# pr0g/ToyMeshPathTracer

Hardware: NVIDIA B200
Metric: Mrays/s (primary+bounce+shadow) (higher is better)
Workload: dtype f32

## Files before the change

toymeshpathtracer_b200/csrc/integrator.cuh:

```cuda
#pragma once
#include "bvh.cuh"

namespace integ {

constexpr int kMaxDepth = 10;
constexpr float kMinT = 0.001f;
constexpr float kMaxT = 1.0e7f;

struct Camera {
    ex::V3 origin, lowerLeftCorner, horizontal, vertical, u, v, w;
    float lensRadius;
};

TMPT_HD void camera_get_ray(const Camera& c, float s, float t, uint32_t& rng, ex::V3& o, ex::V3& d) {
    float px, py;
    ex::random_in_unit_disk(rng, px, py);
    const float rdx = ex::mul(c.lensRadius, px), rdy = ex::mul(c.lensRadius, py);
    const ex::V3 offset = ex::add(ex::muls(c.u, rdx), ex::muls(c.v, rdy));
    o = ex::add(c.origin, offset);
    d = ex::normalize(ex::sub(ex::sub(ex::add(ex::add(c.lowerLeftCorner, ex::muls(c.horizontal, s)), ex::muls(c.vertical, t)), c.origin), offset));
}

TMPT_HD void primary_ray(const Camera& c, int x, int y, float invW, float invH, uint32_t& rng, ex::V3& o, ex::V3& d) {
    const float fv = ex::mul(ex::add((float)y, ex::random_float01(rng)), invH);
    const float fu = ex::mul(ex::add((float)x, ex::random_float01(rng)), invW);
    camera_get_ray(c, fu, fv, rng, o, d);
}

TMPT_HD ex::V3 sky(ex::V3 dir) {
    const float t = ex::mul(0.5f, ex::add(dir.y, 1.0f));
    const float a = ex::sub(1.0f, t);
    return ex::muls(ex::add(ex::v3(ex::mul(1.0f, a), ex::mul(1.0f, a), ex::mul(1.0f, a)), ex::muls(ex::v3(0.5f, 0.7f, 1.0f), t)), 0.5f);
}

TMPT_HD float sun_term(ex::V3 normal, ex::V3 rayDir, ex::V3 lightDir) {
    const ex::V3 nl = ex::dot(normal, rayDir) < 0.0f ? normal : ex::neg(normal);
    return fmaxf(0.0f, ex::dot(lightDir, nl));
}

TMPT_HD ex::V3 scatter_dir(ex::V3 pos, ex::V3 normal, uint32_t& rng) {
    const ex::V3 target = ex::add(ex::add(pos, normal), ex::random_unit_vector(rng));
    return ex::normalize(ex::sub(target, pos));
}

TMPT_HD ex::V3 unwind_step(float k, ex::V3 color) {
    const ex::V3 albedo = ex::v3(0.7f, 0.7f, 0.7f);
    const ex::V3 kLightColor = ex::v3(0.7f, 0.6f, 0.5f);
    const ex::V3 light = ex::add(ex::v3(0.0f, 0.0f, 0.0f), ex::muls(ex::mulv(albedo, kLightColor), k));
    return ex::add(light, ex::mulv(albedo, color));
}

TMPT_HD uchar4 resolve_pixel(ex::V3 sum, float sppRecip) {
    const ex::V3 c = ex::muls(sum, sppRecip);
    uchar4 px;
    px.x = ex::quantise(ex::sqrt_rn(c.x));
    px.y = ex::quantise(ex::sqrt_rn(c.y));
    px.z = ex::quantise(ex::sqrt_rn(c.z));
    px.w = 255;
    return px;
}

struct FirstHit {
    int id;
    float t;
    ex::V3 normal;
};

template <bool STATS = false, bool FAR = true, bool AOV = false, class Stack, class Scene>
TMPT_HD ex::V3 trace_path(Stack& stack, const Scene& sc, const Camera& cam, ex::V3 o, ex::V3 d, ex::V3 lightDir, uint32_t& rng,
                          unsigned long long& rays, bvh::TravStats* stats = nullptr, FirstHit* first = nullptr) {
    float kk[kMaxDepth];
    int depth = 0;
    ex::V3 color = ex::v3(0.0f, 0.0f, 0.0f);
    if (AOV) first->id = -1;
    while (depth < kMaxDepth) {
        ++rays;
        const bvh::HitRec h = bvh::traverse_with<false, STATS, FAR>(stack, sc, o, d, kMinT, kMaxT, stats);
        if (h.id < 0) { color = sky(d); break; }
        ex::V3 pos, normal;
        bvh::hit_payload(sc, h.id, h.u, h.v, pos, normal);
        if (AOV && depth == 0) { first->id = h.id; first->t = h.t; first->normal = normal; }
        ++rays;
#if defined(TMPT_SUN_ONLY) && TMPT_SUN_ONLY
        const bool shadowed = bvh::sun_occluded<STATS>(sc, pos, lightDir, kMinT, kMaxT, stats);
#else
        const bool shadowed = sc.sun.n > 0 ? bvh::sun_occluded<STATS>(sc, pos, lightDir, kMinT, kMaxT, stats)
                                           : bvh::traverse_with<true, STATS, FAR>(stack, sc, pos, lightDir, kMinT, kMaxT, stats).id >= 0;
#endif
        kk[depth] = shadowed ? 0.0f : sun_term(normal, d, lightDir);
        d = scatter_dir(pos, normal, rng);
        o = pos;
        ++depth;
    }
    for (int i = depth - 1; i >= 0; --i) color = unwind_step(kk[i], color);
    return color;
}

constexpr int kMaxChunkSamples = 8;
TMPT_HD int chunk_len(int spp) {
    const int c = spp / 32;
    return c < 1 ? 1 : c > kMaxChunkSamples ? kMaxChunkSamples : c;
}
TMPT_HD int chunk_count(int spp) { const int c = chunk_len(spp); return (spp + c - 1) / c; }

struct AovSums {
    ex::V3 normal;
    float t, hits;
    int id0;
};
TMPT_HD void aov_clear(AovSums& a) { a.normal = ex::v3(0.0f, 0.0f, 0.0f); a.t = 0.0f; a.hits = 0.0f; a.id0 = -1; }
TMPT_HD void aov_add_hit(AovSums& a, ex::V3 normal, float t) { a.normal = ex::add(a.normal, normal); a.t = ex::add(a.t, t); a.hits = ex::add(a.hits, 1.0f); }

TMPT_HD float4 radiance_of(ex::V3 sum, float sppRecip) {
    const ex::V3 c = ex::muls(sum, sppRecip);
    return make_float4(c.x, c.y, c.z, 1.0f);
}
TMPT_HD float4 normal_of(ex::V3 normalSum, float hits, float sppRecip) {
    const ex::V3 n = ex::muls(normalSum, sppRecip);
    return make_float4(n.x, n.y, n.z, ex::mul(hits, sppRecip));
}
TMPT_HD float depth_of(float tSum, float hits) { return hits > 0.0f ? ex::divf(tSum, hits) : ex::u2f(0x7F800000u); }

template <bool STATS = false, bool FAR = true, bool AOV = false, class Stack, class Scene>
TMPT_HD ex::V3 render_chunk(Stack& stack, const Scene& sc, const Camera& cam, int x, int y, int chunk, int width, int height, int spp, int len, ex::V3 lightDir,
                            unsigned long long& rays, bvh::TravStats* stats = nullptr, AovSums* aov = nullptr) {
    const float invW = ex::divf(1.0f, (float)width), invH = ex::divf(1.0f, (float)height);
    uint32_t rng = ex::chunk_seed((uint32_t)chunk, (uint32_t)y * (uint32_t)width + (uint32_t)x, (uint32_t)width * (uint32_t)height);
    ex::V3 sum = ex::v3(0.0f, 0.0f, 0.0f);
    const int s0 = chunk * len, s1 = s0 + len < spp ? s0 + len : spp;
    if (AOV) aov_clear(*aov);
    for (int s = s0; s < s1; ++s) {
        ex::V3 o, d;
        primary_ray(cam, x, y, invW, invH, rng, o, d);
        FirstHit fh;
        sum = ex::add(sum, trace_path<STATS, FAR, AOV>(stack, sc, cam, o, d, lightDir, rng, rays, stats, &fh));
        if (AOV) {
            if (s == s0) aov->id0 = fh.id;
            if (fh.id >= 0) aov_add_hit(*aov, fh.normal, fh.t);
        }
    }
    return sum;
}

TMPT_HD void adaptive_add_chunk(ex::V3 chunkSum, uint32_t& n, float& mean, float& m2) {
    const float y = ex::mul(ex::add(ex::add(ex::mul(0.2126f, chunkSum.x), ex::mul(0.7152f, chunkSum.y)), ex::mul(0.0722f, chunkSum.z)), 0.125f);
    n += 1u;
    const float delta = ex::sub(y, mean);
    mean = ex::add(mean, ex::divf(delta, (float)n));
    m2 = ex::add(m2, ex::mul(delta, ex::sub(y, mean)));
}
TMPT_HD bool adaptive_converged(uint32_t n, float mean, float m2, float tolerance, int minChunks) {
    if (tolerance == 0.0f || n < (uint32_t)minChunks) return false;
    const float a = ex::mul(m2, 65025.0f);
    const float b = ex::mul(ex::mul(ex::mul((float)n, (float)(n - 1u)), ex::mul(4.0f, fmaxf(mean, 0x1p-16f))), ex::mul(tolerance, tolerance));
    return !(a > b);
}

template <bool STATS = false, bool AOV = false, class Scene>
TMPT_HD uchar4 render_pixel(const Scene& sc, const Camera& cam, int x, int y, int width, int height, int spp, ex::V3 lightDir,
                            unsigned long long& rays, ex::V3* outLinear = nullptr, bvh::TravStats* stats = nullptr, AovSums* aov = nullptr) {
    const float sppRecip = ex::divf(1.0f, (float)spp);
    ex::V3 sum = ex::v3(0.0f, 0.0f, 0.0f);
    bvh::LocalStack stack;
    if (AOV) aov_clear(*aov);
    for (int c = 0; c < chunk_count(spp); ++c) {
        AovSums ca;
        sum = ex::add(sum, render_chunk<STATS, true, AOV>(stack, sc, cam, x, y, c, width, height, spp, chunk_len(spp), lightDir, rays, stats, &ca));
        if (AOV) {
            if (c == 0) aov->id0 = ca.id0;
            aov->normal = ex::add(aov->normal, ca.normal); aov->t = ex::add(aov->t, ca.t); aov->hits = ex::add(aov->hits, ca.hits);
        }
    }
    if (outLinear) *outLinear = ex::muls(sum, sppRecip);
    return resolve_pixel(sum, sppRecip);
}

}
```

toymeshpathtracer_b200/csrc/kernels.cu:

```cuda
#include <cooperative_groups.h>
#include <cuda_runtime.h>

#include <atomic>
#include <chrono>
#include <cmath>
#include <cstdarg>
#include <cstdio>
#include <cstdlib>
#include <cstring>
#include <mutex>
#include <new>
#include <string>
#include <vector>

#include "build_logic.cuh"
#include "common.h"
#include "denoise.cuh"
#include "integrator.cuh"
#ifndef TMPT_EXPERIMENTS
#define TMPT_EXPERIMENTS 0
#endif

namespace tmpt {
static thread_local std::string g_err;
// ... 538 lines not shown
                if (h.id >= 0) {
                    if (outT) outT[ray] = h.t;
                    if (outPos || outNormal) {
                        ex::V3 pos, nrm;
                        bvh::hit_payload(sc, h.id, h.u, h.v, pos, nrm);
                        if (outPos) { outPos[ray * 3] = pos.x; outPos[ray * 3 + 1] = pos.y; outPos[ray * 3 + 2] = pos.z; }
                        if (outNormal) { outNormal[ray * 3] = nrm.x; outNormal[ray * 3 + 1] = nrm.y; outNormal[ray * 3 + 2] = nrm.z; }
                    }
                }
            }
            ray = -1;
        }
    }
}
#endif

struct RenderParams {
    bvh::SceneView sc;
    integ::Camera cam;
    ex::V3 lightDir;
    int width, height, spp;
    int stripeRows, rank, world, ownedRows;
    int localWidth;
    int tilesX, numTiles;
    int chunks;
    int chunk0, chunkLen;
    int useAccum;
    float4* sumBuf;
    int bandRow0, bandRows;
    float4* accum;
    uchar4* outStripes;
    uchar4* frame;
    float4* radiance;
    float4* normal;
    float* depth;
    int32_t* triangle;
    unsigned long long* rayCount;
    uint32_t* tileCounter;
    unsigned long long* laneCounter;
    unsigned long long* stats;
    const uint2* list;
    int listLen;
};

__device__ __forceinline__ int owned_row_to_global(int r, int stripeRows, int rank, int world) {
    const int ls = r / stripeRows;
    return (ls * world + rank) * stripeRows + (r - ls * stripeRows);
}
__device__ __forceinline__ bool local_to_global(int xl, int r, int stripeRows, int rank, int world, int width, int& x, int& y) {
    if (stripeRows > 0) {
        x = xl;
        y = owned_row_to_global(r, stripeRows, rank, world);
        return true;
    }
    y = r;
    int t0 = (rank - (r >> 2)) % world;
    t0 += t0 < 0 ? world : 0;
    x = ((t0 + (xl >> 3) * world) << 3) + (xl & 7);
    return x < width;
}

template <int SSTACK, int THREADS>
struct RenderStack {
    using type = bvh::SmemStack<SSTACK, THREADS>;
    static __device__ __forceinline__ type make() {
        extern __shared__ unsigned long long smemStack[];
        return type::make(smemStack, threadIdx.x);
    }
};
template <int THREADS>
struct RenderStack<0, THREADS> {
    using type = bvh::LocalStack;
    static __device__ __forceinline__ type make() { return type(); }
};

#ifndef TMPT_SSTACK
#define TMPT_SSTACK 0
#endif
#ifndef TMPT_TUNE_CFG
#define TMPT_TUNE_CFG 0
#endif
constexpr int kSStack = TMPT_SSTACK;

template <bool STATS, int THREADS, int MINB, int SSTACK, bool FAR = false, bool AOV = false, bool LIST = false>
__global__ void __launch_bounds__(THREADS, MINB) k_render(const RenderParams p) {
    const int lane = threadIdx.x & 31;
    unsigned long long rays = 0;
    bvh::TravStats ts;
    typename RenderStack<SSTACK, THREADS>::type stack = RenderStack<SSTACK, THREADS>::make();
    for (;;) {
        uint32_t tile = 0;
        if (lane == 0) tile = atomicAdd(p.tileCounter, 1u);
        tile = __shfl_sync(0xffffffffu, tile, 0);
        if (tile >= (uint32_t)p.numTiles * (uint32_t)p.chunks) break;
        const int chunk = (int)(tile / (uint32_t)p.numTiles);
        tile -= (uint32_t)chunk * (uint32_t)p.numTiles;
        if (LIST) {
            const uint32_t e = tile * 32u + (uint32_t)lane;
            if (e < (uint32_t)p.listLen) {
                const uint2 en = p.list[e];
                const ex::V3 sum = integ::render_chunk<STATS, FAR>(stack, p.sc, p.cam, (int)(en.x & 0xFFFFu), (int)(en.x >> 16), (int)en.y + chunk, p.width,
                                                                   p.height, 0x7FFFFFFF, integ::kMaxChunkSamples, p.lightDir, rays, &ts);
                __stcs(&p.accum[(size_t)chunk * p.listLen + e], make_float4(sum.x, sum.y, sum.z, 0.0f));
            }
            continue;
        }
        const int tx = (int)(tile % (uint32_t)p.tilesX), ty = (int)(tile / (uint32_t)p.tilesX);
        const int xl = tx * 8 + (lane & 7), rb = ty * 4 + (lane >> 3), r = p.bandRow0 + rb;
        int x, y;
        if (xl < p.localWidth && r < p.ownedRows && local_to_global(xl, r, p.stripeRows, p.rank, p.world, p.width, x, y)) {
            integ::AovSums aov;
            const ex::V3 sum = integ::render_chunk<STATS, FAR, AOV>(stack, p.sc, p.cam, x, y, p.chunk0 + chunk, p.width, p.height, p.spp, p.chunkLen, p.lightDir, rays, &ts, &aov);
            if (AOV && p.triangle && p.chunk0 + chunk == 0) p.triangle[(size_t)y * p.width + x] = aov.id0;
            if (p.useAccum) {
                const size_t a = ((size_t)chunk * p.bandRows + rb) * p.localWidth + xl;
                __stcs(&p.accum[a], make_float4(sum.x, sum.y, sum.z, AOV ? aov.hits : 0.0f));
                if (AOV) __stcs(&p.accum[a + (size_t)p.chunks * p.bandRows * p.localWidth], make_float4(aov.normal.x, aov.normal.y, aov.normal.z, aov.t));
            } else {
                const uchar4 px = integ::resolve_pixel(sum, ex::divf(1.0f, (float)p.spp));
                if (p.frame) p.frame[(size_t)y * p.width + x] = px;
                else p.outStripes[(size_t)r * p.localWidth + xl] = px;
            }
        }
    }
    if (STATS) flush_stats(p.stats, rays, ts, 0);
    for (int o = 16; o > 0; o >>= 1) rays += __shfl_xor_sync(0xffffffffu, rays, o);
    if (lane == 0 && rays) atomicAdd(p.rayCount, rays);
}

#if TMPT_EXPERIMENTS
enum : int { ST_WALK = 0, ST_HIT = 1, ST_SHADOW_DONE = 2, ST_PATH_END = 3, ST_NEED_ITEM = 4, ST_IDLE = 5 };

template <bool STATS, int THREADS, int MINB, int TA, int TB>
__global__ void __launch_bounds__(THREADS, MINB) k_render_regen(const RenderParams p) {
    constexpr unsigned FULL = 0xffffffffu;
    const int lane = threadIdx.x & 31;
    bvh::LocalStack stack;
    float kk[integ::kMaxDepth];
    bvh::WalkState w;
    bvh::TravStats ts;
    w.any = false; w.best.id = -1;
    unsigned long long rays = 0;
    int state = ST_NEED_ITEM;
    bool exhausted = false;
    uint32_t rng = 0;
    int depth = 0, s = 0, sEnd = 0, x = 0, y = 0, xl = 0, rb = 0, chunk = 0;
    ex::V3 sum = ex::v3(0.0f, 0.0f, 0.0f), nd = ex::v3(0.0f, 0.0f, 0.0f);
    float sunk = 0.0f;
    const float invW = ex::divf(1.0f, (float)p.width), invH = ex::divf(1.0f, (float)p.height);
    const unsigned long long totalItems = (unsigned long long)p.numTiles * (unsigned long long)p.chunks * 32ull;
    for (;;) {
        const unsigned notWalking = __ballot_sync(FULL, state != ST_WALK);
        if (notWalking) {
            bool newRay = false, newAny = false;
            ex::V3 no = ex::v3(0.0f, 0.0f, 0.0f), ndir = no;
            const unsigned adv = __ballot_sync(FULL, state == ST_HIT || state == ST_SHADOW_DONE);
            if (adv && (__popc(adv) >= TA || notWalking == FULL)) {
                if (state == ST_HIT) {
                    ex::V3 pos, normal;
                    bvh::hit_payload(p.sc, w.best.id, w.best.u, w.best.v, pos, normal);
                    sunk = integ::sun_term(normal, w.d, p.lightDir);
                    nd = integ::scatter_dir(pos, normal, rng);
                    no = pos; ndir = p.lightDir; newRay = true; newAny = true;
                } else if (state == ST_SHADOW_DONE) {
                    kk[depth] = w.best.id < 0 ? sunk : 0.0f;
                    ++depth;
                    if (depth < integ::kMaxDepth) { no = w.o; ndir = nd; newRay = true; newAny = false; }
                    else state = ST_PATH_END;
                }
            }
            const unsigned endp = __ballot_sync(FULL, state == ST_PATH_END || state == ST_NEED_ITEM);
            const unsigned busy = __ballot_sync(FULL, state == ST_WALK || newRay);
            if (endp && (__popc(endp) >= TB || busy == 0)) {
                if (state == ST_PATH_END) {
                    ex::V3 color = w.any ? ex::v3(0.0f, 0.0f, 0.0f) : integ::sky(w.d);
                    for (int i = depth - 1; i >= 0; --i) color = integ::unwind_step(kk[i], color);
                    sum = ex::add(sum, color);
                    if (++s == sEnd) {
                        if (p.useAccum) {
                            __stcs(&p.accum[((size_t)chunk * p.bandRows + rb) * p.localWidth + xl], make_float4(sum.x, sum.y, sum.z, 0.0f));
                        } else {
                            const uchar4 px = integ::resolve_pixel(sum, ex::divf(1.0f, (float)p.spp));
                            if (p.frame) p.frame[(size_t)y * p.width + x] = px;
                            else p.outStripes[(size_t)(p.bandRow0 + rb) * p.localWidth + xl] = px;
                        }
                        state = ST_NEED_ITEM;
                    }
                }
                const unsigned want = __ballot_sync(FULL, state == ST_NEED_ITEM);
                if (want) {
                    if (exhausted) {
                        if (state == ST_NEED_ITEM) state = ST_IDLE;
                    } else {
                        const int cnt = __popc(want);
                        unsigned long long base = 0;
                        if (lane == 0) base = atomicAdd(p.laneCounter, (unsigned long long)cnt);
                        base = __shfl_sync(FULL, base, 0);
                        exhausted = base + (unsigned long long)cnt >= totalItems;
                        if (state == ST_NEED_ITEM) {
                            const unsigned long long item = base + (unsigned long long)__popc(want & ((1u << lane) - 1u));
                            if (item >= totalItems) {
                                state = ST_IDLE;
                            } else {
                                const uint32_t wi = (uint32_t)(item >> 5), li = (uint32_t)item & 31u;
                                chunk = (int)(wi / (uint32_t)p.numTiles);
                                const uint32_t tile = wi - (uint32_t)chunk * (uint32_t)p.numTiles;
                                const int tx = (int)(tile % (uint32_t)p.tilesX), ty = (int)(tile / (uint32_t)p.tilesX);
                                xl = tx * 8 + (int)(li & 7u); rb = ty * 4 + (int)(li >> 3);
                                const int r = p.bandRow0 + rb;
                                if (xl < p.localWidth && r < p.ownedRows && local_to_global(xl, r, p.stripeRows, p.rank, p.world, p.width, x, y)) {
// ... 1054 lines not shown
        LAUNCH(k_probe_paths, 32, 128, 0, st, s->view, cam, width, height, s->d_probe);
        CU_TRY(cudaMemcpyAsync(s->h_probe, s->d_probe, 4 * sizeof(unsigned int), cudaMemcpyDeviceToHost, st));
        CU_TRY(cudaEventRecord(s->probeDone, st));
        s->probeCam = *camera; s->probeW = width; s->probeH = height;
        s->probePending = true;
        if (s->probeUsePaths < 0) { CU_TRY(cudaEventSynchronize(s->probeDone)); consume(); }
    }
    *usePaths = s->probeUsePaths == 1;
    return TMPT_OK;
}

extern "C" int tmpt_render_kernel_choice(const tmpt_scene* s, int* kernel, float* escapeFraction) {
    if (!s) return tmpt::fail(TMPT_ERR_ARG, "tmpt_render_kernel_choice: NULL scene");
    if (kernel) *kernel = s->lastUsedPaths;
    if (escapeFraction) *escapeFraction = s->probeEscape;
    return TMPT_OK;
}

static int launch_render(const tmpt_scene* cs, const tmpt_camera* camera, int width, int height, int spp, int stripeRows, int rank, int world,
                         uint8_t* outStripes, uint8_t* frame, unsigned long long* rayCountDev, cudaStream_t st,
                         unsigned long long* statsDev = nullptr, const ProgressivePass* prog = nullptr, const FrameOutputs* outs = nullptr) {
    tmpt_scene* s = const_cast<tmpt_scene*>(cs);
    RenderParams p;
    p.sc = s->view;
    static_assert(sizeof(integ::Camera) == sizeof(tmpt_camera), "camera layout");
    memcpy(&p.cam, camera, sizeof p.cam);
    p.lightDir = host_light_dir();
    p.width = width; p.height = height;
    p.spp = prog ? integ::kMaxChunkSamples * (prog->chunk0 + prog->nChunks) : spp;
    p.stripeRows = stripeRows; p.rank = rank; p.world = world;
    p.ownedRows = tmpt_stripe_rows(height, stripeRows, rank, world);
    p.localWidth = tmpt_local_width(width, stripeRows, world);
    p.tilesX = div_up(p.localWidth, 8);
    p.chunks = prog ? prog->nChunks : host_chunk_count(spp);
    p.chunk0 = prog ? prog->chunk0 : 0;
    p.chunkLen = prog ? integ::kMaxChunkSamples : host_chunk_len(spp);
    p.useAccum = (p.chunks > 1 || prog || (outs && outs->accum())) ? 1 : 0;
    const bool aov = outs && outs->aov();
    p.radiance = outs ? outs->radiance : nullptr;
    p.normal = outs ? outs->normal : nullptr;
    p.depth = outs ? outs->depth : nullptr;
    p.triangle = outs ? outs->triangle : nullptr;
    p.sumBuf = prog ? prog->sum : nullptr;
    p.outStripes = (uchar4*)outStripes;
    p.frame = (uchar4*)frame;
    p.rayCount = rayCountDev;
    p.tileCounter = s->d_tileCounter;
    p.laneCounter = s->d_fetchCounter;
    p.stats = statsDev;
    p.accum = nullptr;
    p.list = nullptr;
    p.listLen = 0;
    const AdaptivePass* ad = prog ? prog->adaptive : nullptr;
    const int units = ad ? ad->listLen : p.ownedRows;
    if (units == 0) return TMPT_OK;
    int bandRows = 0;
    const int prc = ad ? prepare_render_chunks(s, 1, p.chunks, true, units, st, &bandRows, 1, 32)
                       : prepare_render_chunks(s, p.localWidth, p.chunks, p.useAccum != 0, p.ownedRows, st, &bandRows, aov ? 2 : 1);
    if (prc != TMPT_OK) return prc;
    p.accum = s->d_accum;
    static const int cfgEnv = getenv("TMPT_RENDER_CFG") ? atoi(getenv("TMPT_RENDER_CFG")) : 0;
    static const int rk = getenv("TMPT_RENDER_KERNEL") ? atoi(getenv("TMPT_RENDER_KERNEL")) : 0;
#if !TMPT_EXPERIMENTS
    if (rk > 0) return tmpt::fail(TMPT_ERR_ARG, "TMPT_RENDER_KERNEL is set, but this library was built without -DTMPT_EXPERIMENTS=1");
#endif
    if (aov && (statsDev || rk > 0 || (TMPT_TUNE_CFG && cfgEnv >= 4)))
        return tmpt::fail(TMPT_ERR_ARG, "render: AOV outputs need the shipped render kernels (no instrumented pass, TMPT_RENDER_KERNEL or tuning configuration)");
    if (ad && (rk > 0 || (TMPT_TUNE_CFG && cfgEnv >= 4)))
        return tmpt::fail(TMPT_ERR_ARG, "render: adaptive passes need the shipped render kernels (no TMPT_RENDER_KERNEL or tuning configuration)");
    constexpr size_t smemPerThread = (size_t)kSStack * sizeof(unsigned long long);
    if (smemPerThread * 256 > 48 * 1024) {
        CU_TRY(cudaFuncSetAttribute(k_render<false, 256, 4, kSStack>, cudaFuncAttributeMaxDynamicSharedMemorySize, (int)(smemPerThread * 256)));
        CU_TRY(cudaFuncSetAttribute(k_render<true, 256, 4, kSStack>, cudaFuncAttributeMaxDynamicSharedMemorySize, (int)(smemPerThread * 256)));
        CU_TRY(cudaFuncSetAttribute(k_render<false, 256, 4, kSStack, false, true>, cudaFuncAttributeMaxDynamicSharedMemorySize, (int)(smemPerThread * 256)));
        CU_TRY(cudaFuncSetAttribute(k_render<false, 256, 4, kSStack, false, false, true>, cudaFuncAttributeMaxDynamicSharedMemorySize, (int)(smemPerThread * 256)));
    }
    if (smemPerThread * 512 > 48 * 1024) {
        CU_TRY(cudaFuncSetAttribute(k_render<false, 512, 2, kSStack>, cudaFuncAttributeMaxDynamicSharedMemorySize, (int)(smemPerThread * 512)));
        CU_TRY(cudaFuncSetAttribute(k_render<false, 512, 2, kSStack, false, true>, cudaFuncAttributeMaxDynamicSharedMemorySize, (int)(smemPerThread * 512)));
        CU_TRY(cudaFuncSetAttribute(k_render<false, 512, 2, kSStack, false, false, true>, cudaFuncAttributeMaxDynamicSharedMemorySize, (int)(smemPerThread * 512)));
    }
    if (smemPerThread * 1024 > 48 * 1024) {
        CU_TRY(cudaFuncSetAttribute(k_render<false, 1024, 1, kSStack>, cudaFuncAttributeMaxDynamicSharedMemorySize, (int)(smemPerThread * 1024)));
        CU_TRY(cudaFuncSetAttribute(k_render<false, 1024, 1, kSStack, false, true>, cudaFuncAttributeMaxDynamicSharedMemorySize, (int)(smemPerThread * 1024)));
        CU_TRY(cudaFuncSetAttribute(k_render<false, 1024, 1, kSStack, false, false, true>, cudaFuncAttributeMaxDynamicSharedMemorySize, (int)(smemPerThread * 1024)));
    }
    const bool farCamera = s->view.farLimit > 0.0f &&
        std::max(std::max(std::fabs(camera->origin[0]), std::fabs(camera->origin[1])), std::fabs(camera->origin[2])) + std::fabs(camera->lensRadius) >
            0.5f * s->view.farLimit;
    if (farCamera && smemPerThread * 256 > 48 * 1024) {
        CU_TRY(cudaFuncSetAttribute(k_render<false, 256, 4, kSStack, true>, cudaFuncAttributeMaxDynamicSharedMemorySize, (int)(smemPerThread * 256)));
        CU_TRY(cudaFuncSetAttribute(k_render<false, 256, 4, kSStack, true, true>, cudaFuncAttributeMaxDynamicSharedMemorySize, (int)(smemPerThread * 256)));
        CU_TRY(cudaFuncSetAttribute(k_render<false, 256, 4, kSStack, true, false, true>, cudaFuncAttributeMaxDynamicSharedMemorySize, (int)(smemPerThread * 256)));
    }
    bool usePaths = false;
    if (!statsDev && !farCamera && rk == 0 && cfgEnv == 0) {
        const int rc = choose_render_kernel(s, camera, p.cam, width, height, st, &usePaths);
        if (rc != TMPT_OK) return rc;
    }
    if (!statsDev) s->lastUsedPaths = usePaths ? 1 : 0;
    int perSMp256 = 0, perSMp1024 = 0;
    if (usePaths) {
        CU_TRY(cudaOccupancyMaxActiveBlocksPerMultiprocessor(&perSMp256, k_render_paths<256, 4, 8>, 256, 0));
        CU_TRY(cudaOccupancyMaxActiveBlocksPerMultiprocessor(&perSMp1024, k_render_paths<1024, 1, 8>, 1024, 0));
    }
#if TMPT_TUNE_CFG
    if (cfgEnv >= 4 && cfgEnv <= 8) {
        for (p.bandRow0 = 0; p.bandRow0 < p.ownedRows; p.bandRow0 += bandRows) {
            const int rowsHere = std::min(bandRows, p.ownedRows - p.bandRow0);
            p.bandRows = rowsHere;
            p.numTiles = p.tilesX * div_up(rowsHere, 4);
            CU_TRY(cudaMemsetAsync(s->d_tileCounter, 0, sizeof(uint32_t), st));
            if (cfgEnv == 4) LAUNCH((k_render<false, 768, 1, 0>), s->smCount, 768, 0, st, p);
            else if (cfgEnv == 5) LAUNCH((k_render<false, 576, 2, 0>), 2 * s->smCount, 576, 0, st, p);
            else if (cfgEnv == 6) LAUNCH((k_render<false, 640, 2, 0>), 2 * s->smCount, 640, 0, st, p);
            else if (cfgEnv == 7) LAUNCH((k_render<false, 896, 1, 0>), s->smCount, 896, 0, st, p);
            else LAUNCH((k_render<false, 384, 3, 0>), 3 * s->smCount, 384, 0, st, p);
            if (p.useAccum) LAUNCH(k_resolve<false>, div_up((long long)rowsHere * p.localWidth, 256), 256, 0, st, p, rowsHere);
        }
        CU_TRY(cudaGetLastError());
        return TMPT_OK;
    }
#endif
    int perSM256 = 0, perSM512 = 0, perSM1024 = 0;
    CU_TRY(cudaOccupancyMaxActiveBlocksPerMultiprocessor(&perSM256, k_render<false, 256, 4, kSStack>, 256, smemPerThread * 256));
    CU_TRY(cudaOccupancyMaxActiveBlocksPerMultiprocessor(&perSM512, k_render<false, 512, 2, kSStack>, 512, smemPerThread * 512));
    CU_TRY(cudaOccupancyMaxActiveBlocksPerMultiprocessor(&perSM1024, k_render<false, 1024, 1, kSStack>, 1024, smemPerThread * 1024));
    for (int b0 = 0; b0 < units; b0 += bandRows) {
        const int rowsHere = std::min(bandRows, units - b0);
        if (ad) {
            p.list = s->d_adList + b0;
            p.listLen = rowsHere;
            p.numTiles = div_up(rowsHere, 32);
        } else {
            p.bandRow0 = b0;
            p.bandRows = rowsHere;
            p.numTiles = p.tilesX * div_up(rowsHere, 4);
        }
        const long long items = (long long)p.numTiles * p.chunks;
        if (items >= 0xFFFFFFFFll) return tmpt::fail(TMPT_ERR_ARG, "render: too many work items in one band");
        CU_TRY(cudaMemsetAsync(s->d_tileCounter, 0, sizeof(uint32_t), st));
        const int cfg = (statsDev || rk > 0 || farCamera) ? 1 : cfgEnv > 0 ? cfgEnv : (items >= (long long)s->smCount * 32 * 8 && perSM1024 > 0) ? 3 : 1;
        const int threads = cfg == 3 ? 1024 : cfg == 2 ? 512 : 256;
        const int perSM = cfg == 3 ? perSM1024 : cfg == 2 ? perSM512 : perSM256;
        const int grid = (int)std::min<long long>((long long)s->smCount * std::max(perSM, 1), (items + threads / 32 - 1) / (threads / 32));
#if TMPT_EXPERIMENTS
        if (rk > 0 && !statsDev) {
            CU_TRY(cudaMemsetAsync(s->d_fetchCounter, 0, sizeof(unsigned long long), st));
            int perSMr = 0;
#define REGEN_CASE(V, TA, TB)                                                                                        \
            if (rk == V) {                                                                                           \
                CU_TRY(cudaOccupancyMaxActiveBlocksPerMultiprocessor(&perSMr, k_render_regen<false, 256, 4, TA, TB>, 256, 0)); \
                const int gridR = (int)std::min<long long>((long long)s->smCount * std::max(perSMr, 1), (items * 32 + 255) / 256); \
                LAUNCH((k_render_regen<false, 256, 4, TA, TB>), gridR, 256, 0, st, p);                                 \
            } else
            REGEN_CASE(1, 8, 4) REGEN_CASE(2, 4, 2) REGEN_CASE(3, 12, 6) REGEN_CASE(4, 16, 4)
#undef REGEN_CASE
#define PATHS_CASE(V, T, MB, GT)                                                                                       \
            if (rk == V) {                                                                                           \
                CU_TRY(cudaOccupancyMaxActiveBlocksPerMultiprocessor(&perSMr, k_render_paths<T, MB, GT>, T, 0));     \
                const int gridR = (int)std::min<long long>((long long)s->smCount * std::max(perSMr, 1), (items * 32 + T - 1) / T); \
                LAUNCH((k_render_paths<T, MB, GT>), gridR, T, 0, st, p);                                              \
            } else
            PATHS_CASE(5, 256, 4, 1) PATHS_CASE(6, 256, 4, 8) PATHS_CASE(7, 256, 4, 16) PATHS_CASE(8, 1024, 1, 8) PATHS_CASE(9, 1024, 1, 16)
#undef PATHS_CASE
            return tmpt::fail(TMPT_ERR_ARG, "TMPT_RENDER_KERNEL=%d: no such render kernel", rk);
        } else
#endif
        if (usePaths) {
            CU_TRY(cudaMemsetAsync(s->d_fetchCounter, 0, sizeof(unsigned long long), st));
            const bool big = items >= (long long)s->smCount * 32 * 8 && perSMp1024 > 0;
            const int t = big ? 1024 : 256;
            const int gridP = (int)std::min<long long>((long long)s->smCount * std::max(big ? perSMp1024 : perSMp256, 1), (items * 32 + t - 1) / t);
            if (ad) {
                if (big) LAUNCH((k_render_paths<1024, 1, 8, false, true>), gridP, 1024, 0, st, p);
                else LAUNCH((k_render_paths<256, 4, 8, false, true>), gridP, 256, 0, st, p);
            } else if (aov) {
                if (big) LAUNCH((k_render_paths<1024, 1, 8, true>), gridP, 1024, 0, st, p);
                else LAUNCH((k_render_paths<256, 4, 8, true>), gridP, 256, 0, st, p);
            } else if (big) LAUNCH((k_render_paths<1024, 1, 8>), gridP, 1024, 0, st, p);
            else LAUNCH((k_render_paths<256, 4, 8>), gridP, 256, 0, st, p);
        } else if (ad) {
            if (farCamera) LAUNCH((k_render<false, 256, 4, kSStack, true, false, true>), grid, 256, smemPerThread * 256, st, p);
            else if (cfg == 3) LAUNCH((k_render<false, 1024, 1, kSStack, false, false, true>), grid, 1024, smemPerThread * 1024, st, p);
            else if (cfg == 2) LAUNCH((k_render<false, 512, 2, kSStack, false, false, true>), grid, 512, smemPerThread * 512, st, p);
            else LAUNCH((k_render<false, 256, 4, kSStack, false, false, true>), grid, 256, smemPerThread * 256, st, p);
        } else if (aov) {
            if (farCamera) LAUNCH((k_render<false, 256, 4, kSStack, true, true>), grid, 256, smemPerThread * 256, st, p);
            else if (cfg == 3) LAUNCH((k_render<false, 1024, 1, kSStack, false, true>), grid, 1024, smemPerThread * 1024, st, p);
            else if (cfg == 2) LAUNCH((k_render<false, 512, 2, kSStack, false, true>), grid, 512, smemPerThread * 512, st, p);
            else LAUNCH((k_render<false, 256, 4, kSStack, false, true>), grid, 256, smemPerThread * 256, st, p);
        } else if (farCamera && !statsDev) LAUNCH((k_render<false, 256, 4, kSStack, true>), grid, 256, smemPerThread * 256, st, p);
        else if (statsDev) LAUNCH((k_render<true, 256, 4, kSStack>), grid, 256, smemPerThread * 256, st, p);
        else if (cfg == 3) LAUNCH((k_render<false, 1024, 1, kSStack>), grid, 1024, smemPerThread * 1024, st, p);
        else if (cfg == 2) LAUNCH((k_render<false, 512, 2, kSStack>), grid, 512, smemPerThread * 512, st, p);
        else LAUNCH((k_render<false, 256, 4, kSStack>), grid, 256, smemPerThread * 256, st, p);
        if (ad) LAUNCH(k_resolve_adaptive, div_up(rowsHere, 256), 256, 0, st, p, prog->sum, s->d_adN, s->d_adStat, ad->tolerance, ad->minChunks, s->d_adActive);
        else if (p.useAccum && aov) LAUNCH(k_resolve<true>, div_up((long long)rowsHere * p.localWidth, 256), 256, 0, st, p, rowsHere);
        else if (p.useAccum) LAUNCH(k_resolve<false>, div_up((long long)rowsHere * p.localWidth, 256), 256, 0, st, p, rowsHere);
    }
    CU_TRY(cudaGetLastError());
    return TMPT_OK;
}

static int check_render_args(const tmpt_scene* s, const tmpt_camera* camera, int width, int height, int spp) {
    if (!s || !camera) return tmpt::fail(TMPT_ERR_ARG, "render: NULL scene / camera");
    if (width < 1 || width > 10000 || height < 1 || height > 10000 || spp < 1 || spp > 1024)
        return tmpt::fail(TMPT_ERR_ARG, "render: width %d height %d spp %d out of range", width, height, spp);
    return TMPT_OK;
}

extern "C" int tmpt_render_stripes(const tmpt_scene* s, const tmpt_camera* camera, int width, int height, int spp, int stripeRows, int rank,
                                   int worldSize, uint8_t* outStripes, uint8_t* peerFrame, uint64_t* rayCountDev, void* stream) {
    int rc = check_render_args(s, camera, width, height, spp);
    if (rc != TMPT_OK) return rc;
    if (stripeRows < 0 || worldSize < 1 || rank < 0 || rank >= worldSize || (!outStripes && !peerFrame) || !rayCountDev)
        return tmpt::fail(TMPT_ERR_ARG, "tmpt_render_stripes: bad stripe arguments");
    DeviceGuard guard(s->device);
    if (!guard.ok) return tmpt::fail(TMPT_ERR_CUDA, "tmpt_render_stripes: cudaSetDevice(%d) failed", s->device);
    return launch_render(s, camera, width, height, spp, stripeRows, rank, worldSize, outStripes, peerFrame,
                         (unsigned long long*)rayCountDev, stream ? (cudaStream_t)stream : s->stream);
}

static int check_outputs(const char* fn, const tmpt_outputs* out, int mem) {
    if (!out) return tmpt::fail(TMPT_ERR_ARG, "%s: out is NULL", fn);
    if (!out->rgba && !out->radiance && !out->normal && !out->depth && !out->triangle) return tmpt::fail(TMPT_ERR_ARG, "%s: no output requested", fn);
    if (mem != TMPT_HOST && mem != TMPT_DEVICE) return tmpt::fail(TMPT_ERR_ARG, "%s: mem %d", fn, mem);
    return TMPT_OK;
}

static int grow_scratch(void** p, size_t* cap, size_t need) {
    if (*cap >= need) return TMPT_OK;
    cudaFree(*p); *p = nullptr; *cap = 0;
    CU_TRY(cudaMalloc(p, need));
    *cap = need;
    return TMPT_OK;
}

static int render_frame(tmpt_scene* s, const tmpt_camera* camera, int width, int height, int spp, int mem, const tmpt_outputs* out,
                        const ProgressivePass* prog, cudaStream_t st, uint64_t* rayCount, double* seconds) {
    const size_t pixels = (size_t)width * height;
    const size_t bytes[5] = {pixels * 4, pixels * sizeof(float4), pixels * sizeof(float4), pixels * sizeof(float), pixels * sizeof(int32_t)};
    void* user[5] = {out->rgba, out->radiance, out->normal, out->depth, out->triangle};
    void* dev[5] = {out->rgba, out->radiance, out->normal, out->depth, out->triangle};
    if (mem == TMPT_HOST || !out->rgba) {
        int rc = grow_scratch((void**)&s->d_frame, &s->frameBytes, bytes[0]);
        if (rc != TMPT_OK) return rc;
        dev[0] = s->d_frame;
    }
    if (mem == TMPT_HOST)
        for (int k = 1; k < 5; ++k)
            if (user[k]) {
                const int rc = grow_scratch(&s->d_outs[k - 1], &s->outsBytes[k - 1], bytes[k]);
                if (rc != TMPT_OK) return rc;
                dev[k] = s->d_outs[k - 1];
            }
    FrameOutputs f;
    f.radiance = (float4*)dev[1]; f.normal = (float4*)dev[2]; f.depth = (float*)dev[3]; f.triangle = (int32_t*)dev[4];
    AdaptivePass* ad = prog ? prog->adaptive : nullptr;
    int32_t* userSamples = ad ? ad->samples : nullptr;
    if (userSamples && mem == TMPT_HOST) {
        const int rc = grow_scratch((void**)&s->d_samples, &s->samplesBytes, pixels * sizeof(int32_t));
        if (rc != TMPT_OK) return rc;
        ad->samples = s->d_samples;
    }
    const int chunks = prog ? prog->nChunks : host_chunk_count(spp);
    int rc = ad ? prepare_render_chunks(s, 1, chunks, true, (int)pixels, st, nullptr, 1, 32)
                : prepare_render_chunks(s, width, chunks, prog || f.accum(), height, st, nullptr, f.aov() ? 2 : 1);
    if (rc != TMPT_OK) return rc;
    CU_TRY(cudaEventRecord(s->ev0, st));
    CU_TRY(cudaMemsetAsync(s->d_rayCount, 0, sizeof(unsigned long long), st));
    if (ad) {
// ... 414 lines not shown
```

Before: 7780.

## Spill per-path state to shared-memory columns to cut register pressure in render kernel

Moves per-path state (work item, pixel coords, sample counter, depth, RNG, running sum, AOV sums) from registers into a per-thread column of static shared memory, accessed through volatile ld/st.shared, and recomputes pixel indices from the stored item after tracing. Ray counts are packed into a control word and accumulated per warp in shared memory rather than held as 64-bit per-thread counters. The aim is fewer live registers across the BVH traversal so more warps stay resident. In exchange it adds many shared-memory loads and stores per bounce, uses shared memory that may compete with the traversal stack, and disables the 1024-thread AOV configuration.

Result: no change. 7786 (median of 6 runs) (+0.1%).

```diff
diff --git a/toymeshpathtracer_b200/csrc/integrator.cuh b/toymeshpathtracer_b200/csrc/integrator.cuh
--- a/toymeshpathtracer_b200/csrc/integrator.cuh
+++ b/toymeshpathtracer_b200/csrc/integrator.cuh
@@ -60,39 +60,92 @@
     return px;
 }
 
-struct FirstHit {
-    int id;
-    float t;
-    ex::V3 normal;
-};
-
-template <bool STATS = false, bool FAR = true, bool AOV = false, class Stack, class Scene>
-TMPT_HD ex::V3 trace_path(Stack& stack, const Scene& sc, const Camera& cam, ex::V3 o, ex::V3 d, ex::V3 lightDir, uint32_t& rng,
-                          unsigned long long& rays, bvh::TravStats* stats = nullptr, FirstHit* first = nullptr) {
+enum : int {
+    kPsItem = 0,
+    kPsXY,
+    kPsCtl,
+    kPsRng,
+    kPsSum,
+    kPathWords = kPsSum + 3,
+    kPsAovNormal = kPathWords,
+    kPsAovT = kPsAovNormal + 3,
+    kPsAovHits,
+    kPsAovId0,
+    kPathWordsAov
+};
+constexpr uint32_t kCtlRays = 0xFFFFu, kCtlDepthShift = 16, kCtlLeftShift = 20, kCtlFirst = 1u << 28;
+
+template <int WORDS>
+struct RegPathState {
+    uint32_t w[WORDS];
+    TMPT_HD void put(int i, uint32_t v) { w[i] = v; }
+    TMPT_HD uint32_t get(int i) const { return w[i]; }
+};
+template <int STRIDE>
+struct ColumnPathState {
+#ifdef __CUDA_ARCH__
+    uint32_t col;
+    __device__ __forceinline__ void put(int i, uint32_t v) {
+        asm volatile("st.shared.u32 [%0], %1;" ::"r"(col + (uint32_t)(i * STRIDE * 4)), "r"(v) : "memory");
+    }
+    __device__ __forceinline__ uint32_t get(int i) const {
+        uint32_t v;
+        asm volatile("ld.shared.u32 %0, [%1];" : "=r"(v) : "r"(col + (uint32_t)(i * STRIDE * 4)) : "memory");
+        return v;
+    }
+#else
+    uint32_t* col;
+    void put(int i, uint32_t v) { col[(size_t)i * STRIDE] = v; }
+    uint32_t get(int i) const { return col[(size_t)i * STRIDE]; }
+#endif
+};
+template <class PS>
+TMPT_HD void ps_put3(PS& ps, int i, ex::V3 v) { ps.put(i, ex::f2u(v.x)); ps.put(i + 1, ex::f2u(v.y)); ps.put(i + 2, ex::f2u(v.z)); }
+template <class PS>
+TMPT_HD ex::V3 ps_get3(const PS& ps, int i) { return ex::v3(ex::u2f(ps.get(i)), ex::u2f(ps.get(i + 1)), ex::u2f(ps.get(i + 2))); }
+
+template <bool STATS = false, bool FAR = true, bool AOV = false, class PS, class Stack, class Scene>
+TMPT_HD ex::V3 trace_path(PS& ps, Stack& stack, const Scene& sc, ex::V3 o, ex::V3 d, ex::V3 lightDir, bvh::TravStats* stats = nullptr) {
     float kk[kMaxDepth];
-    int depth = 0;
     ex::V3 color = ex::v3(0.0f, 0.0f, 0.0f);
-    if (AOV) first->id = -1;
-    while (depth < kMaxDepth) {
-        ++rays;
+    for (;;) {
         const bvh::HitRec h = bvh::traverse_with<false, STATS, FAR>(stack, sc, o, d, kMinT, kMaxT, stats);
-        if (h.id < 0) { color = sky(d); break; }
+        uint32_t ctl = ps.get(kPsCtl) + 1u;
+        const int depth = (int)((ctl >> kCtlDepthShift) & 15u);
+        if (h.id < 0) {
+            ps.put(kPsCtl, ctl);
+            color = sky(d);
+            break;
+        }
         ex::V3 pos, normal;
         bvh::hit_payload(sc, h.id, h.u, h.v, pos, normal);
-        if (AOV && depth == 0) { first->id = h.id; first->t = h.t; first->normal = normal; }
-        ++rays;
+        if (AOV && depth == 0) {
+            if (ctl & kCtlFirst) ps.put(kPsAovId0, (uint32_t)h.id);
+            ps_put3(ps, kPsAovNormal, ex::add(ps_get3(ps, kPsAovNormal), normal));
+            ps.put(kPsAovT, ex::f2u(ex::add(ex::u2f(ps.get(kPsAovT)), h.t)));
+            ps.put(kPsAovHits, ex::f2u(ex::add(ex::u2f(ps.get(kPsAovHits)), 1.0f)));
+        }
+        ps.put(kPsCtl, ctl + 1u);
+        const float k = sun_term(normal, d, lightDir);
 #if defined(TMPT_SUN_ONLY) && TMPT_SUN_ONLY
         const bool shadowed = bvh::sun_occluded<STATS>(sc, pos, lightDir, kMinT, kMaxT, stats);
 #else
         const bool shadowed = sc.sun.n > 0 ? bvh::sun_occluded<STATS>(sc, pos, lightDir, kMinT, kMaxT, stats)
                                            : bvh::traverse_with<true, STATS, FAR>(stack, sc, pos, lightDir, kMinT, kMaxT, stats).id >= 0;
 #endif
-        kk[depth] = shadowed ? 0.0f : sun_term(normal, d, lightDir);
+        ctl = ps.get(kPsCtl);
+        const int dk = (int)((ctl >> kCtlDepthShift) & 15u);
+        kk[dk] = shadowed ? 0.0f : k;
+        uint32_t rng = ps.get(kPsRng);
         d = scatter_dir(pos, normal, rng);
+        ps.put(kPsRng, rng);
         o = pos;
-        ++depth;
-    }
-    for (int i = depth - 1; i >= 0; --i) color = unwind_step(kk[i], color);
+        ps.put(kPsCtl, ctl + (1u << kCtlDepthShift));
+        if (dk + 1 == kMaxDepth) break;
+    }
+    const uint32_t ctl = ps.get(kPsCtl);
+    for (int i = (int)((ctl >> kCtlDepthShift) & 15u) - 1; i >= 0; --i) color = unwind_step(kk[i], color);
+    ps.put(kPsCtl, ctl & ~(15u << kCtlDepthShift));
     return color;
 }
 
@@ -121,25 +174,43 @@
 }
 TMPT_HD float depth_of(float tSum, float hits) { return hits > 0.0f ? ex::divf(tSum, hits) : ex::u2f(0x7F800000u); }
 
+template <bool STATS = false, bool FAR = true, bool AOV = false, class PS, class Stack, class Scene>
+TMPT_HD ex::V3 render_chunk(PS& ps, Stack& stack, const Scene& sc, const Camera& cam, int x, int y, int chunk, int width, int height, int spp, int len,
+                            ex::V3 lightDir, unsigned long long& rays, bvh::TravStats* stats = nullptr, AovSums* aov = nullptr) {
+    ps.put(kPsXY, (uint32_t)x | ((uint32_t)y << 16));
+    ps.put(kPsRng, ex::chunk_seed((uint32_t)chunk, (uint32_t)y * (uint32_t)width + (uint32_t)x, (uint32_t)width * (uint32_t)height));
+    const int s0 = chunk * len, s1 = s0 + len < spp ? s0 + len : spp;
+    ps.put(kPsCtl, s1 > s0 ? ((uint32_t)(s1 - s0) << kCtlLeftShift) | kCtlFirst : 0u);
+    ps_put3(ps, kPsSum, ex::v3(0.0f, 0.0f, 0.0f));
+    if (AOV) {
+        AovSums a;
+        aov_clear(a);
+        ps_put3(ps, kPsAovNormal, a.normal);
+        ps.put(kPsAovT, ex::f2u(a.t)); ps.put(kPsAovHits, ex::f2u(a.hits)); ps.put(kPsAovId0, (uint32_t)a.id0);
+    }
+    while (ps.get(kPsCtl) >> kCtlLeftShift) {
+        const float invW = ex::divf(1.0f, (float)width), invH = ex::divf(1.0f, (float)height);
+        const uint32_t xy = ps.get(kPsXY);
+        uint32_t rng = ps.get(kPsRng);
+        ex::V3 o, d;
+        primary_ray(cam, (int)(xy & 0xFFFFu), (int)(xy >> 16), invW, invH, rng, o, d);
+        ps.put(kPsRng, rng);
+        const ex::V3 c = trace_path<STATS, FAR, AOV>(ps, stack, sc, o, d, lightDir, stats);
+        ps_put3(ps, kPsSum, ex::add(ps_get3(ps, kPsSum), c));
+        ps.put(kPsCtl, (ps.get(kPsCtl) - (1u << kCtlLeftShift)) & ~kCtlFirst);
+    }
+    rays += ps.get(kPsCtl) & kCtlRays;
+    if (AOV) {
+        aov->normal = ps_get3(ps, kPsAovNormal);
+        aov->t = ex::u2f(ps.get(kPsAovT)); aov->hits = ex::u2f(ps.get(kPsAovHits)); aov->id0 = (int)ps.get(kPsAovId0);
+    }
+    return ps_get3(ps, kPsSum);
+}
 template <bool STATS = false, bool FAR = true, bool AOV = false, class Stack, class Scene>
 TMPT_HD ex::V3 render_chunk(Stack& stack, const Scene& sc, const Camera& cam, int x, int y, int chunk, int width, int height, int spp, int len, ex::V3 lightDir,
                             unsigned long long& rays, bvh::TravStats* stats = nullptr, AovSums* aov = nullptr) {
-    const float invW = ex::divf(1.0f, (float)width), invH = ex::divf(1.0f, (float)height);
-    uint32_t rng = ex::chunk_seed((uint32_t)chunk, (uint32_t)y * (uint32_t)width + (uint32_t)x, (uint32_t)width * (uint32_t)height);
-    ex::V3 sum = ex::v3(0.0f, 0.0f, 0.0f);
-    const int s0 = chunk * len, s1 = s0 + len < spp ? s0 + len : spp;
-    if (AOV) aov_clear(*aov);
-    for (int s = s0; s < s1; ++s) {
-        ex::V3 o, d;
-        primary_ray(cam, x, y, invW, invH, rng, o, d);
-        FirstHit fh;
-        sum = ex::add(sum, trace_path<STATS, FAR, AOV>(stack, sc, cam, o, d, lightDir, rng, rays, stats, &fh));
-        if (AOV) {
-            if (s == s0) aov->id0 = fh.id;
-            if (fh.id >= 0) aov_add_hit(*aov, fh.normal, fh.t);
-        }
-    }
-    return sum;
+    RegPathState<AOV ? kPathWordsAov : kPathWords> ps;
+    return render_chunk<STATS, FAR, AOV>(ps, stack, sc, cam, x, y, chunk, width, height, spp, len, lightDir, rays, stats, aov);
 }
 
 TMPT_HD void adaptive_add_chunk(ex::V3 chunkSum, uint32_t& n, float& mean, float& m2) {
diff --git a/toymeshpathtracer_b200/csrc/kernels.cu b/toymeshpathtracer_b200/csrc/kernels.cu
--- a/toymeshpathtracer_b200/csrc/kernels.cu
+++ b/toymeshpathtracer_b200/csrc/kernels.cu
@@ -644,50 +644,75 @@
 #endif
 constexpr int kSStack = TMPT_SSTACK;
 
+template <int WORDS, int THREADS>
+__device__ __forceinline__ integ::ColumnPathState<THREADS> path_state() {
+    __shared__ uint32_t words[WORDS * THREADS];
+    integ::ColumnPathState<THREADS> ps;
+    ps.col = (uint32_t)__cvta_generic_to_shared(words) + threadIdx.x * 4u;
+    return ps;
+}
+
+__device__ __forceinline__ bool render_item_pixel(const RenderParams& p, uint32_t item, int lane, int& chunk, int& xl, int& rb, int& r, int& x, int& y) {
+    chunk = (int)(item / (uint32_t)p.numTiles);
+    const uint32_t tile = item - (uint32_t)chunk * (uint32_t)p.numTiles;
+    const int tx = (int)(tile % (uint32_t)p.tilesX), ty = (int)(tile / (uint32_t)p.tilesX);
+    xl = tx * 8 + (lane & 7); rb = ty * 4 + (lane >> 3); r = p.bandRow0 + rb;
+    return xl < p.localWidth && r < p.ownedRows && local_to_global(xl, r, p.stripeRows, p.rank, p.world, p.width, x, y);
+}
+
 template <bool STATS, int THREADS, int MINB, int SSTACK, bool FAR = false, bool AOV = false, bool LIST = false>
 __global__ void __launch_bounds__(THREADS, MINB) k_render(const RenderParams p) {
+    __shared__ unsigned long long warpRays[THREADS / 32];
     const int lane = threadIdx.x & 31;
-    unsigned long long rays = 0;
+    unsigned long long statRays = 0;
     bvh::TravStats ts;
     typename RenderStack<SSTACK, THREADS>::type stack = RenderStack<SSTACK, THREADS>::make();
+    auto ps = path_state<AOV ? integ::kPathWordsAov : integ::kPathWords, THREADS>();
+    if (lane == 0) warpRays[threadIdx.x >> 5] = 0;
     for (;;) {
-        uint32_t tile = 0;
-        if (lane == 0) tile = atomicAdd(p.tileCounter, 1u);
-        tile = __shfl_sync(0xffffffffu, tile, 0);
-        if (tile >= (uint32_t)p.numTiles * (uint32_t)p.chunks) break;
-        const int chunk = (int)(tile / (uint32_t)p.numTiles);
-        tile -= (uint32_t)chunk * (uint32_t)p.numTiles;
+        uint32_t item = 0;
+        if (lane == 0) item = atomicAdd(p.tileCounter, 1u);
+        item = __shfl_sync(0xffffffffu, item, 0);
+        if (item >= (uint32_t)p.numTiles * (uint32_t)p.chunks) break;
+        ps.put(integ::kPsItem, item);
+        unsigned long long rays = 0;
         if (LIST) {
-            const uint32_t e = tile * 32u + (uint32_t)lane;
+            const int chunk = (int)(item / (uint32_t)p.numTiles);
+            const uint32_t e = (item - (uint32_t)chunk * (uint32_t)p.numTiles) * 32u + (uint32_t)lane;
             if (e < (uint32_t)p.listLen) {
                 const uint2 en = p.list[e];
-                const ex::V3 sum = integ::render_chunk<STATS, FAR>(stack, p.sc, p.cam, (int)(en.x & 0xFFFFu), (int)(en.x >> 16), (int)en.y + chunk, p.width,
-                                                                   p.height, 0x7FFFFFFF, integ::kMaxChunkSamples, p.lightDir, rays, &ts);
-                __stcs(&p.accum[(size_t)chunk * p.listLen + e], make_float4(sum.x, sum.y, sum.z, 0.0f));
+                const ex::V3 sum = integ::render_chunk<STATS, FAR>(ps, stack, p.sc, p.cam, (int)(en.x & 0xFFFFu), (int)(en.x >> 16), (int)en.y + chunk,
+                                                                   p.width, p.height, 0x7FFFFFFF, integ::kMaxChunkSamples, p.lightDir, rays, &ts);
+                const uint32_t it = ps.get(integ::kPsItem), ch = it / (uint32_t)p.numTiles;
+                __stcs(&p.accum[(size_t)ch * p.listLen + (it - ch * (uint32_t)p.numTiles) * 32u + (uint32_t)(threadIdx.x & 31)],
+                       make_float4(sum.x, sum.y, sum.z, 0.0f));
             }
-            continue;
-        }
-        const int tx = (int)(tile % (uint32_t)p.tilesX), ty = (int)(tile / (uint32_t)p.tilesX);
-        const int xl = tx * 8 + (lane & 7), rb = ty * 4 + (lane >> 3), r = p.bandRow0 + rb;
-        int x, y;
-        if (xl < p.localWidth && r < p.ownedRows && local_to_global(xl, r, p.stripeRows, p.rank, p.world, p.width, x, y)) {
-            integ::AovSums aov;
-            const ex::V3 sum = integ::render_chunk<STATS, FAR, AOV>(stack, p.sc, p.cam, x, y, p.chunk0 + chunk, p.width, p.height, p.spp, p.chunkLen, p.lightDir, rays, &ts, &aov);
-            if (AOV && p.triangle && p.chunk0 + chunk == 0) p.triangle[(size_t)y * p.width + x] = aov.id0;
-            if (p.useAccum) {
-                const size_t a = ((size_t)chunk * p.bandRows + rb) * p.localWidth + xl;
-                __stcs(&p.accum[a], make_float4(sum.x, sum.y, sum.z, AOV ? aov.hits : 0.0f));
-                if (AOV) __stcs(&p.accum[a + (size_t)p.chunks * p.bandRows * p.localWidth], make_float4(aov.normal.x, aov.normal.y, aov.normal.z, aov.t));
-            } else {
-                const uchar4 px = integ::resolve_pixel(sum, ex::divf(1.0f, (float)p.spp));
-                if (p.frame) p.frame[(size_t)y * p.width + x] = px;
-                else p.outStripes[(size_t)r * p.localWidth + xl] = px;
+        } else {
+            int chunk, xl, rb, r, x, y;
+            if (render_item_pixel(p, item, lane, chunk, xl, rb, r, x, y)) {
+                integ::AovSums aov;
+                const ex::V3 sum = integ::render_chunk<STATS, FAR, AOV>(ps, stack, p.sc, p.cam, x, y, p.chunk0 + chunk, p.width, p.height, p.spp, p.chunkLen,
+                                                                        p.lightDir, rays, &ts, &aov);
+                render_item_pixel(p, ps.get(integ::kPsItem), threadIdx.x & 31, chunk, xl, rb, r, x, y);
+                if (AOV && p.triangle && p.chunk0 + chunk == 0) p.triangle[(size_t)y * p.width + x] = aov.id0;
+                if (p.useAccum) {
+                    const size_t a = ((size_t)chunk * p.bandRows + rb) * p.localWidth + xl;
+                    __stcs(&p.accum[a], make_float4(sum.x, sum.y, sum.z, AOV ? aov.hits : 0.0f));
+                    if (AOV) __stcs(&p.accum[a + (size_t)p.chunks * p.bandRows * p.localWidth], make_float4(aov.normal.x, aov.normal.y, aov.normal.z, aov.t));
+                } else {
+                    const uchar4 px = integ::resolve_pixel(sum, ex::divf(1.0f, (float)p.spp));
+                    if (p.frame) p.frame[(size_t)y * p.width + x] = px;
+                    else p.outStripes[(size_t)r * p.localWidth + xl] = px;
+                }
             }
         }
-    }
-    if (STATS) flush_stats(p.stats, rays, ts, 0);
-    for (int o = 16; o > 0; o >>= 1) rays += __shfl_xor_sync(0xffffffffu, rays, o);
-    if (lane == 0 && rays) atomicAdd(p.rayCount, rays);
+        if (STATS) statRays += rays;
+        uint32_t n = (uint32_t)rays;
+        for (int o = 16; o > 0; o >>= 1) n += __shfl_xor_sync(0xffffffffu, n, o);
+        if ((threadIdx.x & 31) == 0) warpRays[threadIdx.x >> 5] += n;
+    }
+    if (STATS) flush_stats(p.stats, statRays, ts, 0);
+    if ((threadIdx.x & 31) == 0 && warpRays[threadIdx.x >> 5]) atomicAdd(p.rayCount, warpRays[threadIdx.x >> 5]);
 }
 
 #if TMPT_EXPERIMENTS
@@ -1908,7 +1933,6 @@
     }
     if (smemPerThread * 1024 > 48 * 1024) {
         CU_TRY(cudaFuncSetAttribute(k_render<false, 1024, 1, kSStack>, cudaFuncAttributeMaxDynamicSharedMemorySize, (int)(smemPerThread * 1024)));
-        CU_TRY(cudaFuncSetAttribute(k_render<false, 1024, 1, kSStack, false, true>, cudaFuncAttributeMaxDynamicSharedMemorySize, (int)(smemPerThread * 1024)));
         CU_TRY(cudaFuncSetAttribute(k_render<false, 1024, 1, kSStack, false, false, true>, cudaFuncAttributeMaxDynamicSharedMemorySize, (int)(smemPerThread * 1024)));
     }
     const bool farCamera = s->view.farLimit > 0.0f &&
@@ -1966,7 +1990,8 @@
         const long long items = (long long)p.numTiles * p.chunks;
         if (items >= 0xFFFFFFFFll) return tmpt::fail(TMPT_ERR_ARG, "render: too many work items in one band");
         CU_TRY(cudaMemsetAsync(s->d_tileCounter, 0, sizeof(uint32_t), st));
-        const int cfg = (statsDev || rk > 0 || farCamera) ? 1 : cfgEnv > 0 ? cfgEnv : (items >= (long long)s->smCount * 32 * 8 && perSM1024 > 0) ? 3 : 1;
+        int cfg = (statsDev || rk > 0 || farCamera) ? 1 : cfgEnv > 0 ? cfgEnv : (items >= (long long)s->smCount * 32 * 8 && perSM1024 > 0) ? 3 : 1;
+        if (aov && cfg == 3) cfg = 2;
         const int threads = cfg == 3 ? 1024 : cfg == 2 ? 512 : 256;
         const int perSM = cfg == 3 ? perSM1024 : cfg == 2 ? perSM512 : perSM256;
         const int grid = (int)std::min<long long>((long long)s->smCount * std::max(perSM, 1), (items + threads / 32 - 1) / (threads / 32));
@@ -2013,7 +2038,6 @@
             else LAUNCH((k_render<false, 256, 4, kSStack, false, false, true>), grid, 256, smemPerThread * 256, st, p);
         } else if (aov) {
             if (farCamera) LAUNCH((k_render<false, 256, 4, kSStack, true, true>), grid, 256, smemPerThread * 256, st, p);
-            else if (cfg == 3) LAUNCH((k_render<false, 1024, 1, kSStack, false, true>), grid, 1024, smemPerThread * 1024, st, p);
             else if (cfg == 2) LAUNCH((k_render<false, 512, 2, kSStack, false, true>), grid, 512, smemPerThread * 512, st, p);
             else LAUNCH((k_render<false, 256, 4, kSStack, false, true>), grid, 256, smemPerThread * 256, st, p);
         } else if (farCamera && !statsDev) LAUNCH((k_render<false, 256, 4, kSStack, true>), grid, 256, smemPerThread * 256, st, p);
```
